# liulab-dfci/TRUST4

Measured on AMD Instinct MI355X. Metric: stage-1 assembly read pairs/sec (150 bp PE), whole stage 1, higher is better.
Workload: dtype int32/u64

## Files before the change

### trust4_amd/csrc/t4_api.hip

```cpp
#include <hip/hip_runtime.h>
#include <math.h>
#include <stdarg.h>
#include <stdio.h>
#include <string.h>
#include <zlib.h>

#include <algorithm>
#include <atomic>
#include <chrono>
#include <map>
#include <memory>
#include <mutex>
#include <string>
#include <thread>
#include <unordered_map>
#include <vector>

#ifdef __HIPCC__
#include <dlfcn.h>
#include <rccl/rccl.h>
#include <type_traits>
#include <unistd.h>
#endif
#include "../../include/trust4_hip.h"
// ... 293 lines not shown
    while (n < groups) n *= 2;
    if (c->grpPoolHost) (void)hipHostFree(c->grpPoolHost);
    c->grpPoolHost = nullptr; w.grpPool = nullptr; w.grpCap = 0;
    HIPCHK(c, hipHostMalloc(&c->grpPoolHost, sizeof(T4Grp) * 2 * (size_t)n, hipHostMallocMapped));
    HIPCHK(c, hipHostGetDevicePointer((void **)&w.grpPool, c->grpPoolHost, 0));
    w.grpCap = n;
  }
  return T4_OK;
}
T4Wide wideHalf(const t4_ctx *c, int half) {
  T4Wide w = c->wide;
  if (!half) return w;
  const size_t R = (size_t)w.maxReads, P = (size_t)w.maxPart;
  w.seed += R * T4_WIDE_SEEDS; w.bounds += R * (T4_WIDE_MAXP + 1); w.uniqPref += R * (w.pcap + 1); w.sortTmp += R * 2 * w.pcap; w.requeue += R; w.headBits += R * ((w.pcap + 31) / 32);
  w.pCnt += P; w.pRead += P; w.pKeys += P * w.pcap; w.gSize += P * w.pcap; w.gInfo += P * w.pcap; w.gCount += P * 4; w.gOff += P * 2;
  w.pRec += P * w.maxOvPart * 10; w.pRecCnt += P; w.mKeys += P * w.maxOvPart; w.mOrd += P * w.maxOvPart;
  w.grpPool += w.grpCap;
  return w;
}

}

extern "C" {

int t4_init(int device_ordinal, t4_ctx **out) {
  if (!out) return T4_ERR_ARG;
  *out = nullptr;
  int ndev = 0;
  if (hipGetDeviceCount(&ndev) != hipSuccess || ndev <= 0 || device_ordinal < 0 || device_ordinal >= ndev) return T4_ERR_HIP;
  if (hipSetDevice(device_ordinal) != hipSuccess) return T4_ERR_HIP;
  t4_ctx *c = new t4_ctx();
  c->device = device_ordinal;
  hipDeviceProp_t prop;
  if (hipGetDeviceProperties(&prop, device_ordinal) != hipSuccess) { delete c; return T4_ERR_HIP; }
  c->cus = prop.multiProcessorCount;
  if (hipStreamCreate(&c->stream) != hipSuccess) { delete c; return T4_ERR_HIP; }
  for (int i = 0; i < 4; ++i) if (hipEventCreate(&c->ev[i]) != hipSuccess) { delete c; return T4_ERR_HIP; }
  memset(&c->stats, 0, sizeof c->stats);
  if (hipMalloc(&c->listCounts, sizeof(int) * 16) != hipSuccess || hipMalloc(&c->hitCounter, sizeof(unsigned long long)) != hipSuccess) { delete c; return T4_ERR_HIP; }
  if (hipHostMalloc(&c->aqFlagHost, 64, hipHostMallocMapped) != hipSuccess || hipHostGetDevicePointer((void **)&c->aqFlagDev, c->aqFlagHost, 0) != hipSuccess ||
      hipMalloc(&c->aqDoneCtr, sizeof(unsigned)) != hipSuccess || hipMemset(c->aqDoneCtr, 0, sizeof(unsigned)) != hipSuccess) { delete c; return T4_ERR_HIP; }
  *c->aqFlagHost = 0;
  *out = c;
  return T4_OK;
}

void t4_destroy(t4_ctx *c) {
  if (!c) return;
  (void)hipSetDevice(c->device);
#ifdef T4_PHASE_TIMING
  if (getenv("T4_PHASE_DUMP")) {
    unsigned long long ph[T4_NPHASE];
    if (hipMemcpyFromSymbol(ph, HIP_SYMBOL(t4k::g_phaseCycles), sizeof(ph)) == hipSuccess) {
      static const char *names[32] = {"other", "seed:lookup", "expand", "sort", "stats", "runs", "bigsort", "chain", "ovsort", "score", "prefilter", "final", "annotate", "score:quick", "score:banded", "score:finish", "extend:ungapped", "after-extend", "extend:list", "extend:dp4", "extend:dp1", "extend:combine", "seed:replay", "seed:scan", "extend:launch", "-", "-", "-", "-", "-", "-", "-"};
      unsigned long long tot = 0;
      for (int i = 0; i < T4_NPHASE; ++i) tot += ph[i];
      for (int i = 0; i < T4_NPHASE; ++i) if (ph[i]) fprintf(stderr, "phase %-16s %-7s %6.2f%%  %.3e cycles\n", names[i & 31], i < 32 ? "lds" : "global", 100.0 * (double)ph[i] / (double)tot, (double)ph[i]);
    }
    static unsigned long long cls[4 * T4_NPHASE];
    if (hipMemcpyFromSymbol(cls, HIP_SYMBOL(t4k::g_phaseByOverlaps), sizeof(cls)) == hipSuccess) {
      static const char *names[32] = {"other", "seed:lookup", "expand", "sort", "stats", "runs", "bigsort", "chain", "ovsort", "score", "prefilter", "final", "annotate", "score:quick", "score:banded", "score:finish", "extend:ungapped", "after-extend", "extend:list", "extend:dp4", "extend:dp1", "extend:combine", "seed:replay", "seed:scan", "extend:launch", "-", "-", "-", "-", "-", "-", "-"};
      static const char *cname[4] = {"<5 overlaps", "5-19 overlaps", "20-64 overlaps", ">64 overlaps"};
      for (int k = 0; k < 4; ++k) {
        unsigned long long tot = 0;
        for (int i = 0; i < T4_NPHASE; ++i) tot += cls[k * T4_NPHASE + i];
        if (!tot) continue;
        fprintf(stderr, "AddRead queries with %s: %.3e cycles in the query kernel\n", cname[k], (double)tot);
        for (int i = 0; i < T4_NPHASE; ++i) if (cls[k * T4_NPHASE + i] * 200 >= tot) fprintf(stderr, "   %-16s %-7s %6.2f%%\n", names[i & 31], i < 32 ? "lds" : "global", 100.0 * (double)cls[k * T4_NPHASE + i] / (double)tot);
      }
    }
    unsigned long long dc[8];
    if (hipMemcpyFromSymbol(dc, HIP_SYMBOL(t4k::g_dbgCount), sizeof(dc)) == hipSuccess)
      fprintf(stderr, "debug counters: gap jobs %llu, banded %llu, wave-DP steps %llu, scratch fallbacks %llu; overhang DPs %llu, of which %llu leave the diagonal\n", dc[0], dc[1], dc[2], dc[3], dc[6], dc[7]);
  }
#endif
  void *ptrs[] = {c->dpRows, c->dpDir, c->gKeys, c->gPairs, c->gCand, c->gOv, c->gFin, c->gOrd, c->hitsKeys, c->lists,
                  c->listCounts, c->status, c->counts, c->hitCounter, c->result, c->aqIn, c->aqOut};
  if (c->aqInHost) (void)hipHostFree(c->aqInHost);
  if (c->aqOutHost) (void)hipHostFree(c->aqOutHost);
  if (c->aqFlagHost) (void)hipHostFree(c->aqFlagHost);
  if (c->aqDoneCtr) (void)hipFree(c->aqDoneCtr);
  if (c->aqPool) (void)hipHostFree(c->aqPool);
  if (c->candPool) (void)hipHostFree(c->candPool);
  if (c->aqRecDev) (void)hipFree(c->aqRecDev);
  if (c->aqRecRead) (void)hipFree(c->aqRecRead);
  if (c->aqExtAux) (void)hipFree(c->aqExtAux);
  if (c->wideInit) {
    void *wp[] = {c->wide.seed, c->wide.bounds, c->wide.pCnt, c->wide.pRead, c->wide.pKeys, c->wide.gSize, c->wide.gInfo, c->wide.gCount, c->wide.gOff, c->wide.pRec,
                  c->wide.pRecCnt, c->wide.uniqPref, c->wide.mKeys, c->wide.mOrd, c->wide.sortTmp, c->wide.requeue};
    for (void *p : wp) if (p) (void)hipFree(p);
    if (c->grpPoolHost) (void)hipHostFree(c->grpPoolHost);
    if (c->headBitsHost) (void)hipHostFree(c->headBitsHost);
  }
  for (void *p : ptrs) if (p) (void)hipFree(p);
  for (int i = 0; i < 4; ++i) if (c->ev[i]) (void)hipEventDestroy(c->ev[i]);
  if (c->stream) (void)hipStreamDestroy(c->stream);
  if (c->stream2) (void)hipStreamDestroy(c->stream2);
  if (c->evIn) (void)hipEventDestroy(c->evIn);
  if (c->evG) (void)hipEventDestroy(c->evG);
  delete c;
}

int t4_sync(t4_ctx *c) {
  if (!c) return T4_ERR_ARG;
  HIPCHK(c, hipStreamSynchronize(c->stream));
  return T4_OK;
}
const char *t4_last_error(t4_ctx *c) { return c ? c->err.c_str() : "null ctx"; }
int t4_device_cus(t4_ctx *c) { return c ? c->cus : 0; }
int t4_ctx_device(t4_ctx *c) { return c ? c->device : 0; }
#ifdef T4_PHASE_TIMING
int t4_debug_phase_cycles(unsigned long long *out16) {
  unsigned long long zero[T4_NPHASE] = {0};
  if (hipMemcpyFromSymbol(out16, HIP_SYMBOL(t4k::g_phaseCycles), sizeof(zero)) != hipSuccess) return T4_ERR_HIP;
// ... 2696 lines not shown
```

### trust4_amd/csrc/t4_kernels.h

```cpp
#pragma once
#include <hip/hip_runtime.h>

#include "t4_device.h"

namespace t4k {

#ifdef T4_INLINE_ALL
#define T4_NI
#else
#define T4_NI __attribute__((noinline))
#endif
#ifndef T4_OPT_JOBSORT
#define T4_OPT_JOBSORT 1
#endif
#ifndef T4_OPT_ROWWALK
#define T4_OPT_ROWWALK 1
#endif
#ifndef T4_NI_R3
#define T4_NI_R3 0
#endif
#ifdef __HIPCC__
#define T4_LDS_AS __attribute__((address_space(3)))
#else
#define T4_LDS_AS
// ... 2737 lines not shown
    if (f == i) {
      slotOf[i] = k;
      if (gt == 3 && cSlot < 0) cSlot = k;
      kept[k++] = oi;
    } else if (f < i && gt == 2) {
      const int used = slotOf[f];
      const OvRec &base = wm.fin[kept[used]];
      if (o.matchCnt == base.matchCnt && ovSimDen(o) == ovSimDen(base) && cSlot >= 0) {
        const OvRec &c = wm.fin[kept[cSlot]];
        if (o.re <= c.rs + 3) {
          int d1 = o.re - c.rs, d2 = base.re - c.rs;
          if (d1 < 0) d1 = -d1;
          if (d2 < 0) d2 = -d2;
          if (base.re > c.rs + 3 || d1 < d2) kept[used] = oi;
        }
      }
    }
  }
  if (k > 0) {
    char BT = 0, chain = 0;
    for (int i = 0; i < k; ++i) {
      const OvRec &o = wm.fin[kept[i]];
      char n0 = OV_NAME0(o.flags), n2 = OV_NAME2(o.flags);
      if (BT && n0 != BT) continue;
      BT = n0;
      if (chain && !(n2 == chain || (n2 == 'D' && chain == 'A') || (n2 == 'A' && chain == 'D'))) continue;
      chain = n2;
      int gt = OV_GENETYPE(o.flags) == 255 ? -1 : OV_GENETYPE(o.flags);
      if (gt >= 0 && g[gt] == -1) g[gt] = kept[i];
    }
    if (g[3] != -1) {
      const OvRec &c = wm.fin[g[3]];
      if (c.re - c.rs + 1 <= readLen / 2 && c.re - c.rs + 1 <= 50) {
        for (int i = 0; i < 3; ++i) {
          if (g[i] < 0) continue;
          const OvRec &x = wm.fin[g[i]];
          if ((x.re - 17 > c.rs || c.re < x.re) && c.ss >= 100) { g[3] = -1; break; }
        }
      }
    }
  }
  for (int t = 0; t < 4; ++t) {
    if (g[t] >= 0) storeOverlap(out + t, wm.fin[g[t]]);
    else {
      T4OverlapOut z;
      z.seqIdx = -1; z.readStart = z.readEnd = z.seqStart = z.seqEnd = -1; z.strand = 1; z.matchCnt = 0; z.indelCnt = 0; z.similarity = 0;
      out[t] = z;
    }
  }
}

struct ExtSide { short size, good, match, mis, indel, pending; };
struct ExtOut { int ret, rs, re, ss, se, matchCnt, simFail, den; };

#define T4_EXT_BYTES(L) (((L) + 1) * 11 + 3 * (L) + 8)
#define T4_EXT_WST(buf, L) ((buf) + ((L) + 1) * 11 + 2 * (L) + 8)
#define PS_INDEL (1u << 27)
__device__ __forceinline__ unsigned pathStepDiag(unsigned s, bool eq) {
  if (s & PS_INDEL) return s;
  unsigned good = s & 511u, tmp = (s >> 9) & 511u, k = ((s >> 18) & 511u) + 1u;
  if (eq) { ++tmp; if (4u * tmp > 3u * k) good = k; }
  return good | tmp << 9 | k << 18;
}
__device__ __forceinline__ unsigned pathBorder(int n) {
  const unsigned one = 1u | 1u << 9 | 1u << 18;
  return n == 1 ? one : (one | PS_INDEL);
}
__device__ unsigned dpWaveTracePW(const T4PW *w, int L, const char *p, unsigned char *dirbuf) {
  const int d = laneId(), W = 11, leftBand = 5;
  unsigned char *wst = T4_EXT_WST(dirbuf, L);
  for (int t = d; t < L; t += 64) wst[t] = w[t];
  waveLdsSync();
  const int negInf = (L + 1) * (L + 1) * (-4);
  int M = negInf;
  unsigned S = PS_INDEL, fin = PS_INDEL;
  { int j0 = d - leftBand; if (d < W && j0 >= 0 && j0 <= L) M = j0 == 0 ? 0 : -4 - 4 * j0; }
  const int lastStep = 2 * L + W - 1;
  for (int s = 2; s <= lastStep; ++s) {
    int lM = waveUp1(M), uM = waveDown1(M);
    const unsigned lS = waveUp1(S), uS = waveDown1(S);
    const int i2 = s - d, i = i2 >> 1, j = i - leftBand + d;
    if (d < W && (i2 & 1) == 0 && i >= 1 && i <= L && j >= 1 && j <= L) {
      if (j == 1) lM = -4 - 4 * i; else if (d == 0) lM = negInf;
      if (i == 1) uM = -4 - 4 * j; else if (d + 1 >= W) uM = negInf;
      int dM;
      if (i == 1) dM = (j - 1 == 0) ? 0 : -4 - 4 * (j - 1);
      else if (j == 1) dM = -4 - 4 * (i - 1);
      else dM = M;
      const bool eq = baseEqualW(wst[j - 1], p[i - 1]);
      const int dsc = dM + (eq ? 2 : -2);
      int m = dsc;
      if (lM - 4 > m) m = lM - 4;
      if (uM - 4 > m) m = uM - 4;
      dirbuf[i * W + d] = (unsigned char)((lM - 4 == m ? 1 : 0) | (uM - 4 == m ? 2 : 0) | (dsc == m ? 4 : 0) | (eq ? 8 : 0));
      if (dsc == m) S = pathStepDiag((i == 1 && j == 1) ? 0u : ((i == 1 || j == 1) ? pathBorder(i + j - 2) : S), eq);
      else if (uM - 4 == m) S = (i == 1 ? pathBorder(j) : uS) | PS_INDEL;
      else S = (j == 1 ? pathBorder(i) : lS) | PS_INDEL;
      if (i == L && j == L) fin = S;
      M = m;
    }
  }
  return (unsigned)__shfl((int)fin, leftBand);
}
__device__ unsigned dpRowTracePW(const T4PW *w, int L, const char *p, unsigned char *dirbuf, int Lmax) {
  const int d = laneId() & 15, W = 11, leftBand = 5;
  unsigned char *wst = T4_EXT_WST(dirbuf, L);
// ... 56 lines not shown
      if (i == 1) uM = -4 - 4 * j; else if (last) uM = (neg_);                                                                         \
      const int dM = i == 1 ? (j == 1 ? 0 : -4 * j) : (j == 1 ? -4 * i : Mself);                                                       \
      const bool eq = baseEqualW((w_)[j - 1], (p_)[i - 1]);                                                                            \
      const int dsc = dM + (eq ? 2 : -2);                                                                                              \
      int m = dsc;                                                                                                                     \
      if (lM - 4 > m) m = lM - 4;                                                                                                      \
      if (uM - 4 > m) m = uM - 4;                                                                                                      \
      if (dsc == m) { Sself = pathStepDiag((i == 1 && j == 1) ? 0u : ((i == 1 || j == 1) ? pathBorder(i + j - 2) : Sself), eq); Rself = (i == 1 ? 0 : Rself) + 1; } \
      else if (uM - 4 == m) { Sself = (i == 1 ? pathBorder(j) : uS) | PS_INDEL; Rself = 0; }                                           \
      else { Sself = (j == 1 ? pathBorder(i) : lS) | PS_INDEL; Rself = 0; }                                                            \
      Mself = m;                                                                                                                       \
    }                                                                                                                                  \
  }
  for (int u = 0; u < nPair; ++u) {
    T4_PAIR_STEP(ME, MO, SE, SO, RE, LE, wE, pE, negE, iE)
    T4_PAIR_STEP(MO, ME, SO, SE, RO, LO, wO, pO, negO, iO)
    ++iE; ++iO;
  }
#undef T4_PAIR_STEP
  const int src = (laneId() & ~15) + leftBand;
  const unsigned sA = (unsigned)__shfl((int)SO, src), sB = (unsigned)__shfl((int)SE, src);
  const unsigned rA = (unsigned)__shfl(RO, src), rB = (unsigned)__shfl(RE, src);
  outA = (unsigned long long)sA | ((unsigned long long)rA << 32);
  outB = (unsigned long long)sB | ((unsigned long long)rB << 32);
}
__device__ int tracebackPW(const unsigned char *dirbuf, int L, signed char *align) {
  const int W = 11, leftBand = 5;
  int tagi = L, tagj = L, tag = 0;
  while (tagi > 0 || tagj > 0) {
    int a = 0;
    if (tagi > 0 && tagj > 0) {
      unsigned char bits = dirbuf[tagi * W + (tagj - tagi + leftBand)];
      if (bits & 1) a = 3;
      if (bits & 2) a = 2;
      if (bits & 4) a = (bits & 8) ? 0 : 1;
    } else if (tagi == 0) {
      int mL = (tagj - 1 == 0) ? 0 : (-4 - 4 * (tagj - 1));
      if (mL - 4 == -4 - 4 * tagj) a = 3;
    } else {
      int mU = (tagi - 1 == 0) ? 0 : (-4 - 4 * (tagi - 1));
      if (mU - 4 == -4 - 4 * tagi) a = 2;
    }
    align[tag++] = (signed char)a;
    if (a == 3) --tagj; else if (a == 2) --tagi; else { --tagi; --tagj; }
  }
  for (int i = 0, j = tag - 1; i < j; ++i, --j) { signed char x = align[i]; align[i] = align[j]; align[j] = x; }
  return tag;
}

__device__ void extendOverlaps(const T4IndexView &ix, WaveMem &wm, WaveState *ws, int n, int len, bool useFirstStrand,
                               double factor, ExtSide *sides, unsigned char *dirbuf, int dirBytes, ExtOut *res, bool lean = false) {
  const int lane = tid(), NT = nthr();
  const int plus0 = n > 0 ? (wm.fin[wm.ord[0]].flags & OV_PLUS) : 1;
  {
    const int wave = lane >> 6, nwv = NT >> 6, wl = lane & 63;
    for (int q = wave; q < 2 * n; q += nwv) {
      const OvRec &o = wm.fin[wm.ord[q >> 1]];
      const int side = q & 1;
      const T4SeqInfo si = ix.seqs[o.seqIdx];
      const char *r = (useFirstStrand ? plus0 : (o.flags & OV_PLUS)) ? wm.seg : wm.rc;
      int size, t0, p0;
      if (side == 0) { size = o.rs < o.ss ? o.rs : o.ss; t0 = o.ss - size; p0 = o.rs - size; }
      else { int a = len - 1 - o.re, b = si.len - 1 - o.se; size = a < b ? a : b; t0 = o.se + 1; p0 = o.re + 1; }
      const T4PW *w = ix.pw + si.pwOff + t0;
      int mm = 0, good = 0, tmpBase = 0;
      for (int base = 0; base < size; base += 64) {
        const int k = base + wl;
        const int pos = side == 0 ? size - 1 - k : k;
        const bool in = k < size;
        const bool eq = in && baseEqualW(w[pos], r[p0 + pos]);
        const unsigned long long bal = __ballot(eq);
        const int tmp = tmpBase + __popcll(bal & ((wl == 63) ? ~0ull : ((2ull << wl) - 1ull)));
        const unsigned long long gb = __ballot(eq && tmp > 0.75 * (k + 1));
        if (gb) good = base + 64 - __clzll((long long)gb);
        mm += __popcll(__ballot(in && !eq));
        tmpBase += __popcll(bal);
      }
      if (wl == 0) {
        ExtSide e;
        e.size = (short)size; e.match = (short)(size - mm); e.mis = (short)mm; e.indel = 0; e.pending = 0;
        if (size > 1 && !((size - mm) * 2 - mm * 2 >= size * 2 - 8)) e.pending = 1;
        e.good = (short)good;
        sides[q] = e;
      }
    }
  }
  __syncthreads();
  PHASE_MARK(ws, 18);
  if (lean) {
    int nPend = 0, maxL = 0;
    for (int q0 = 0; q0 < 2 * n; q0 += NT) {
      const int q = q0 + lane;
      const bool pend = q < 2 * n && sides[q].pending;
      int tot;
      const int inc = blockInclScan(pend ? 1 : 0, ws->red, tot);
      if (pend) wm.cand[nPend + inc - 1] = (unsigned)q;
      nPend += tot;
      int mx;
      blockInclMaxScan(pend ? (int)sides[q].size : 0, ws->red, mx);
      if (mx > maxL) maxL = mx;
    }
    __syncthreads();
    PHASE_MARK(ws, 19);
    const int nw = NT >> 6, slice = (maxL + 15) & ~15;
    int perChunk = nw * 8;
    if (slice > 0 && perChunk * slice > dirBytes) perChunk = (dirBytes / slice) & ~7;
    if (nPend > 0 && perChunk < 8) { if (lane == 0) ws->unsupported = 1; nPend = 0; }
    const int wave = lane >> 6, wl = lane & 63, row = wl >> 4, l16 = wl & 15;
    for (int c0 = 0; c0 < nPend; c0 += perChunk) {
      int Lq[2] = {0, 0}, qq[2] = {-1, -1};
      const unsigned char *wst[2] = {dirbuf, dirbuf};
      const char *pr[2] = {wm.seg, wm.seg};
      for (int z = 0; z < 2; ++z) {
        const int slot = wave * 8 + row * 2 + z, t = c0 + slot;
        if (slot < perChunk && t < nPend) {
          const int q = (int)wm.cand[t];
          const OvRec &o = wm.fin[wm.ord[q >> 1]];
          const int side = q & 1, L = sides[q].size;
          const T4SeqInfo si = ix.seqs[o.seqIdx];
          const char *r = (useFirstStrand ? plus0 : (o.flags & OV_PLUS)) ? wm.seg : wm.rc;
          const T4PW *w = ix.pw + si.pwOff + (side == 0 ? o.ss - L : o.se + 1);
          unsigned char *dst = dirbuf + (size_t)slot * slice;
          for (int x = l16; x < L; x += 16) dst[x] = w[x];
          Lq[z] = L; qq[z] = q; wst[z] = dst; pr[z] = r + (side == 0 ? o.rs - L : o.re + 1);
        }
      }
      waveLdsSync();
      int Lmax = Lq[0] > Lq[1] ? Lq[0] : Lq[1];
      { int x = __shfl_xor(Lmax, 16); if (x > Lmax) Lmax = x; x = __shfl_xor(Lmax, 32); if (x > Lmax) Lmax = x; }
      unsigned long long out[2];
      dpRowPairLean(wst[0], Lq[0], pr[0], wst[1], Lq[1], pr[1], Lmax, out[0], out[1]);
      for (int z = 0; z < 2; ++z) {
        const bool have = qq[z] >= 0;
        const unsigned pst = (unsigned)out[z];
        const int q = have ? qq[z] : 0, side = q & 1, L = Lq[z];
        const bool gapped = have && (pst & PS_INDEL) != 0;
        DBG_ADD(6, (have && l16 == 0) ? 1 : 0); DBG_ADD(7, (gapped && l16 == 0) ? 1 : 0);
        const int run = (gapped && side == 0) ? (int)(out[z] >> 32) : 0;
        int runMax = run;
        { int x = __shfl_xor(runMax, 16); if (x > runMax) runMax = x; x = __shfl_xor(runMax, 32); if (x > runMax) runMax = x; }
        int good = 0, tmpBase = 0;
        for (int base = 0; base < runMax; base += 16) {
          const int k = base + l16;
          const bool eq = k < run && baseEqualW(wst[z][L - 1 - k], pr[z][L - 1 - k]);
          const unsigned bal = (unsigned)((__ballot(eq) >> (wl & 48)) & 0xFFFFull);
          const int tmp = tmpBase + __popc(bal & ((2u << l16) - 1u));
          const unsigned gb = (unsigned)((__ballot(eq && 4 * tmp > 3 * (k + 1)) >> (wl & 48)) & 0xFFFFull);
          if (gb) good = base + 32 - __clz(gb);
          tmpBase += __popc(bal);
        }
        if (gapped && side == 1) good = (int)(pst & 511u);
        if (have && l16 == 0) {
          ExtSide e = sides[q];
          if (gapped) { e.match = 0; e.mis = 0; e.indel = 1; e.good = (short)good; }
          e.pending = 0;
          sides[q] = e;
        }
      }
      __syncthreads();
    }
    PHASE_MARK(ws, 21);
  } else {
  const int nwE = NT >> 6, perChunk = nwE * 4;
  const int qslice = (dirBytes / perChunk) & ~15;
  int nFit = 0, nPendSides = 0;
  for (int part = 0; part < 2; ++part) {
    for (int q0 = 0; q0 < 2 * n; q0 += NT) {
      const int q = q0 + lane;
      bool pend = q < 2 * n && sides[q].pending;
      if (pend) { const int size = sides[q].size; const bool fitsQ = T4_EXT_BYTES(size) <= qslice; pend = (part == 0) == fitsQ; }
      int tot;
      const int inc = blockInclScan(pend ? 1 : 0, ws->red, tot);
      if (pend) wm.cand[nPendSides + inc - 1] = (unsigned)q;
      nPendSides += tot;
    }
    if (part == 0) nFit = nPendSides;
  }
  __syncthreads();
  auto finishSide = [&](int q, const signed char *align, int alen) {
    const int side = q & 1;
    int m = 0, mm = 0, ind = 0, good = 0, tmp = 0;
    for (int k = 0; k < alen; ++k) { if (align[k] == 0) ++m; else if (align[k] == 1) ++mm; else ++ind; }
    if (side == 0) {
      for (int i = alen - 1, k = 1; i >= 0; --i, ++k) {
        if (align[i] == 0) { ++tmp; if (tmp > 0.75 * k) good = k; }
        else if (align[i] != 1) break;
      }
    } else {
      for (int i = 0; i < alen; ++i) {
        if (align[i] == 0) { ++tmp; if (tmp > 0.75 * (i + 1)) good = i + 1; }
        else if (align[i] != 1) break;
      }
    }
    ExtSide e = sides[q];
    e.match = (short)m; e.mis = (short)mm; e.indel = (short)ind; e.good = (short)good; e.pending = 0;
    sides[q] = e;
  };
  auto leanSide = [&](int q, const unsigned char *buf, int L, signed char *align) {
    const int side = q & 1;
    int good = 0, tmp = 0;
    if (side == 0) {
      const int W = 11, leftBand = 5;
      int tagi = L, tagj = L, k = 0;
      while (tagi > 0 && tagj > 0) {
        const unsigned char bits = buf[tagi * W + (tagj - tagi + leftBand)];
        if (!(bits & 4)) break;
        ++k;
        if (bits & 8) { ++tmp; if (tmp > 0.75 * k) good = k; }
        --tagi; --tagj;
      }
    } else {
      const int alen = tracebackPW(buf, L, align);
      for (int i = 0; i < alen; ++i) {
        if (align[i] == 0) { ++tmp; if (tmp > 0.75 * (i + 1)) good = i + 1; }
        else if (align[i] != 1) break;
// ... 521 lines not shown
    if (VARIANT == 2) {
      if (SHARED_ARGS) { __syncthreads(); if (threadIdx.x == 0) s_ix = qa.views[qa.viewOf[r]]; __syncthreads(); }
      else ix = qa.views[qa.viewOf[r]];
    }
#ifdef __HIPCC__
    const unsigned long long tick0 = (VARIANT == 1 && qa.readTicks) ? wall_clock64() : 0ull;
#endif
    bool done = processRead<(VARIANT == 0 ? 0 : VARIANT == 3 ? 3 : 1)>(ix, bv, wk, qa, wm, &s_ws, r, sc);
    if (CAP == 8192 && VARIANT == 1 && !done && wk.gKeys) {
      WaveMem wgLocal;
      WaveMem &wg = SHARED_ARGS ? s_wg : wgLocal;
      __syncthreads();
      if (!SHARED_ARGS || threadIdx.x == 0) {
        wg = wm;
        const size_t b = blockIdx.x;
        wg.keys = wk.gKeys + b * (size_t)wk.gCap;
        wg.pairs = wk.gPairs + b * (size_t)wk.gCap * 2;
        wg.cand = wg.pairs + wk.gCap;
        wg.ov = (OvRec *)(wk.gOv + b * (size_t)wk.gMaxOv * 10);
        wg.fin = (OvRec *)(wk.gFin + b * (size_t)wk.gMaxOv * 10);
        wg.ord = wk.gOrd + b * (size_t)wk.gMaxOv;
        wg.cap = wk.gCap; wg.maxOv = wk.gMaxOv; wg.maxFin = wk.gMaxOv; wg.candCap = wk.gCap; wg.ldsArrays = 0; wg.hitLimit = wk.gCap;
        wg.ldsSort = s_keys; wg.ldsSortCap = C;
        wg.dirBuf = (unsigned char *)s_keys; wg.dirBytes = C * 8;
        if (wk.capLimit > 0 && wk.capLimit < C) { int bsz = 64; while (bsz * 2 <= wk.capLimit) bsz *= 2; wg.ldsSortCap = bsz; }
      }
      __syncthreads();
      done = processRead<1>(ix, bv, wk, qa, wg, &s_ws, r, sc);
      if (tid() == 0 && done && wk.nextCount) atomicAdd(wk.nextCount + 2, 1);
    }
    if (tid() == 0) {
#ifdef __HIPCC__
      if (VARIANT == 1 && qa.readTicks) qa.readTicks[r] = (int)(wall_clock64() - tick0);
#endif
#ifdef T4_PHASE_TIMING
      if (VARIANT == 1 && qa.mode == 4) {
        const int nOv = qa.counts[r], cls = nOv < 5 ? 0 : nOv < 20 ? 1 : nOv <= 64 ? 2 : 3;
        for (int p_ = 0; p_ < T4_NPHASE; ++p_) if (s_ws.phaseLocal[p_]) { atomicAdd(&g_phaseByOverlaps[cls * T4_NPHASE + p_], (unsigned long long)s_ws.phaseLocal[p_]); s_ws.phaseLocal[p_] = 0; }
      }
#endif
      if (!done) {
        if (wk.nextList) { int slot = atomicAdd(wk.nextCount, 1); wk.nextList[slot] = (int)r; }
        else wk.status[r] = 2;
      }
      s_nextW = wk.workNext ? (int)gridDim.x + atomicAdd(wk.workNext, 1) : w + (int)gridDim.x;
    }
    __syncthreads();
    w = s_nextW;
    __syncthreads();
  }
}

#ifndef T4_EXT_NREC
#define T4_EXT_NREC 4
#endif
__global__ __launch_bounds__(64) void extendKernel(T4IndexView ix, T4BatchView bv, T4QueryArgs qa, int recBegin) {
  __shared__ OvRec s_fin[T4_EXT_NREC];
  __shared__ unsigned short s_ord[T4_EXT_NREC];
  __shared__ ExtSide s_sides[2 * T4_EXT_NREC];
  __shared__ ExtOut s_res[T4_EXT_NREC];
  __shared__ unsigned s_cand[2 * T4_EXT_NREC + 2];
  __shared__ unsigned long long s_dir[1024];
  __shared__ char s_seg[T4_MAXL + 8];
  __shared__ char s_rc[T4_MAXL + 8];
  __shared__ WaveState s_ws;
  WaveMem wm;
  wm.keys = s_dir; wm.pairs = (unsigned *)s_sides; wm.ov = (OvRec *)s_res; wm.fin = s_fin; wm.ord = s_ord; wm.cand = s_cand;
  wm.seg = s_seg; wm.rc = s_rc;
  wm.cap = 1024; wm.maxOv = T4_EXT_NREC; wm.maxFin = T4_EXT_NREC; wm.candCap = 2 * T4_EXT_NREC + 2; wm.ldsArrays = 1;
  wm.ldsSort = nullptr; wm.ldsSortCap = 0; wm.hitLimit = 0; wm.dirBuf = (unsigned char *)s_dir; wm.dirBytes = (int)sizeof s_dir;
  const int lane = tid();
  const int nRec = (int)*qa.poolCursor < qa.poolCap ? (int)*qa.poolCursor : qa.poolCap;
  for (int g = recBegin + (int)blockIdx.x * T4_EXT_NREC; g < nRec; g += (int)gridDim.x * T4_EXT_NREC) {
    int i0 = g;
    const int gEnd = g + T4_EXT_NREC < nRec ? g + T4_EXT_NREC : nRec;
    while (i0 < gEnd) {
      const int r = qa.recRead[i0];
      int i1 = i0 + 1;
      while (i1 < gEnd && qa.recRead[i1] == r) ++i1;
      if (r < 0) { i0 = i1; continue; }
      const int n = i1 - i0, len = bv.len[r];
      if (lane == 0) { s_ws.overflow = 0; s_ws.unsupported = 0; }
#ifdef T4_PHASE_TIMING
      if (lane == 0) { s_ws.phaseT0 = clock64(); s_ws.phaseBase = 0; s_ws.curPhase = 24; }
#endif
      loadSegment(bv, r, 0, len, wm);
      if (lane < n) {
        const T4OverlapOut t = qa.outDev[i0 + lane];
        OvRec o;
        o.seqIdx = t.seqIdx; o.rs = t.readStart; o.re = t.readEnd; o.ss = t.seqStart; o.se = t.seqEnd;
        o.matchCnt = t.matchCnt; o.indelCnt = t.indelCnt; o.chainPos = 0; o.chainLen = 0;
        o.flags = t.strand == 1 ? OV_PLUS : 0;
        s_fin[lane] = o; s_ord[lane] = (unsigned short)lane;
      }
      __syncthreads();
      extendOverlaps(ix, wm, &s_ws, n, len, false, qa.factorPerRead[r], s_sides, (unsigned char *)s_dir, (int)sizeof s_dir, s_res, qa.leanExt != 0);
      if (lane < n) {
        const T4OverlapOut in = qa.outDev[i0 + lane];
        const ExtOut e = s_res[lane];
        T4OverlapOut t;
        t.seqIdx = in.seqIdx; t.readStart = e.rs; t.readEnd = e.re; t.seqStart = e.ss; t.seqEnd = e.se;
        t.strand = in.strand; t.matchCnt = e.matchCnt;
        if (e.simFail) { t.indelCnt = in.indelCnt; t.similarity = in.similarity; }
        else { t.indelCnt = 0; t.similarity = (double)t.matchCnt / (double)e.den; }
        qa.outExt[i0 + lane] = t;
        qa.ret[i0 + lane] = e.ret;
        if (qa.cs && qa.cs->extAux) qa.cs->extAux[i0 + lane] = e.simFail ? 0 : e.den;
      }
      if (lane == 0 && s_ws.unsupported) qa.poolCursor[1] = 1u;
      __syncthreads();
      i0 = i1;
    }
  }
}

struct PickBest { int idx, seqIdx, rs, re, ss, se, matchCnt, flags; };
__device__ __forceinline__ OvRec pickRec(const PickBest &b) {
  OvRec o;
  o.seqIdx = b.seqIdx; o.rs = b.rs; o.re = b.re; o.ss = b.ss; o.se = b.se; o.matchCnt = b.matchCnt; o.indelCnt = 0; o.chainPos = 0; o.chainLen = 0; o.flags = b.flags;
  return o;
}
__device__ __forceinline__ PickBest pickLoad(const T4OverlapOut *ov, int i) {
  const T4OverlapOut t = ov[i];
  PickBest b;
  b.idx = i; b.seqIdx = t.seqIdx; b.rs = t.readStart; b.re = t.readEnd; b.ss = t.seqStart; b.se = t.seqEnd; b.matchCnt = t.matchCnt;
  b.flags = (t.strand == 1 ? OV_PLUS : 0) | (t.similarity == 0 ? OV_SIMZERO : 0);
  return b;
}
__device__ __forceinline__ bool pickBefore(const PickBest &a, const PickBest &b) {
  const int cm = ovCmp(pickRec(a), pickRec(b), true);
  return cm < 0 || (cm == 0 && a.idx < b.idx);
}
__device__ __forceinline__ PickBest pickShflXor(const PickBest &b, int d) {
  PickBest o;
  o.idx = __shfl_xor(b.idx, d); o.seqIdx = __shfl_xor(b.seqIdx, d); o.rs = __shfl_xor(b.rs, d); o.re = __shfl_xor(b.re, d);
  o.ss = __shfl_xor(b.ss, d); o.se = __shfl_xor(b.se, d); o.matchCnt = __shfl_xor(b.matchCnt, d); o.flags = __shfl_xor(b.flags, d);
  return o;
}
__device__ __forceinline__ PickBest pickReduce(PickBest b, bool wantLast, PickBest *red) {
  for (int d = 32; d > 0; d >>= 1) {
    const PickBest o = pickShflXor(b, d);
    if (o.idx >= 0 && (b.idx < 0 || pickBefore(o, b) != wantLast)) b = o;
  }
  const int wave = threadIdx.x >> 6, nw = (blockDim.x + 63) >> 6;
  if (laneId() == 0) red[wave] = b;
  __syncthreads();
  b = red[0];
  for (int w = 1; w < nw; ++w) {
    const PickBest o = red[w];
    if (o.idx >= 0 && (b.idx < 0 || pickBefore(o, b) != wantLast)) b = o;
  }
  __syncthreads();
  return b;
}
#define T4_PICK_THREADS 256
__global__ __launch_bounds__(T4_PICK_THREADS) void assignPickKernel(int nReads, const int *counts, const int *outBase, const int *lens,
                                                                    const T4OverlapOut *ov, const T4OverlapOut *ext, const int *ret, const int *extAux,
                                                                    int poolCap, int *outRet, T4OverlapOut *out) {
  __shared__ PickBest s_red[T4_PICK_THREADS / 64];
  const int lane = tid(), NT = nthr();
  for (int r = blockIdx.x; r < nReads; r += gridDim.x) {
    const int len = lens[r];
    int n = counts[r], base = n > 0 ? outBase[r] : 0;
    if (n < 0 || base < 0 || base > poolCap) n = 0;
    if (n > poolCap - base) n = poolCap - base;
// ... 637 lines not shown
```

### trust4_amd/csrc/t4_wide.h

```cpp
#pragma once

#define T4_WIDE_SEEDS (2 * T4_MAXL + 2)
#define T4_WIDE_OVBITS 9
#define T4_WIDE_PART_SAMPLES 256

__device__ T4_NI void wideDeferRead(const T4IndexView &ix, WaveMem &wm, WaveState *ws, const T4Wide &wd, int len, int strandArg, long long r,
                                    unsigned long long &hitTotal, int pass, int barcode) {
  const int lane = tid(), NT = nthr();
  unsigned *posStart = (unsigned *)wm.ov, *posPref = wm.pairs;
  const int nk = len - ix.k + 1;
  __syncthreads();
  const int H = seedPositionsNovel(ix, wm, len, strandArg, barcode, pass == 1, posStart, posPref, ws->red, wm.keys, (WaveState *)0);
  hitTotal += (unsigned long long)H;
  int huge = 0;
  if (barcode == -1) for (int q = lane; q < 2 * nk; q += NT) if (posPref[q + 1] - posPref[q] > 10000u) huge = 1;
  huge = blockSum(huge, ws->red) != 0;
  if (lane == 0) {
    int slot = atomicAdd(&wd.ctl[0], 1), pBase = 0, P = 0;
    if (slot >= wd.maxReads) { atomicOr(&wd.ctl[2], 1); slot = -1; }
    else {
      const long long per = 16LL * wd.pcap;
      long long want = ((long long)H * wd.safetyNum + per - 1) / per;
      const int nseq = ix.nseq > 0 ? ix.nseq : 1;
      if (want < 1) want = 1;
// ... 389 lines not shown
      run += tot;
    }
    if (lane == 0) { up[0] = 0; st[WS_M] = lim; }
    __syncthreads();
    unsigned *hb = wd.headBits + (size_t)w * ((wd.pcap + 31) / 32);
    for (int j = lane; j < (lim + 31) / 32; j += NT) {
      unsigned v = 0;
      for (int b = 0; b < 32 && j * 32 + b < lim; ++b) v |= (unsigned)(up[j * 32 + b + 1] - up[j * 32 + b]) << b;
      hb[j] = v;
    }
  }
}

template <int PCAP, int MAXOV>
__global__ __launch_bounds__(512) void wideChainKernel(T4IndexView ixArg, T4BatchView bvArg, T4Work wkArg, T4QueryArgs qaArg, T4Wide wd) {
  __shared__ unsigned long long s_keys[PCAP];
  __shared__ unsigned s_pairs[PCAP + PCAP / 3 + 2];
  __shared__ OvRec s_ov[MAXOV];
  __shared__ unsigned short s_ord[MAXOV];
  __shared__ char s_seg[T4_MAXL + 8];
  __shared__ char s_rc[T4_MAXL + 8];
  __shared__ WaveState s_ws;
  __shared__ T4IndexView s_ix;
  __shared__ T4BatchView s_bv;
  __shared__ T4Work s_wk;
  __shared__ T4QueryArgs s_qa;
  __shared__ WaveMem s_wm;
  if (wd.ctl[2]) return;
  if (threadIdx.x == 0) {
    s_ix = ixArg; s_bv = bvArg; s_wk = wkArg; s_qa = qaArg;
    WaveMem &m = s_wm;
    m.keys = s_keys; m.pairs = s_pairs; m.cand = s_pairs + PCAP; m.ov = s_ov; m.fin = s_ov; m.ord = s_ord;
    m.cap = PCAP; m.maxOv = MAXOV; m.maxFin = MAXOV; m.candCap = PCAP / 3 + 2; m.ldsArrays = 1; m.hitLimit = PCAP;
    m.ldsSort = nullptr; m.ldsSortCap = 0; m.dirBuf = (unsigned char *)s_keys; m.dirBytes = PCAP * 8;
    m.seg = s_seg; m.rc = s_rc;
  }
  __syncthreads();
  const T4IndexView &ix = s_ix;
  const T4BatchView &bv = s_bv;
  const T4Work &wk = s_wk;
  WaveMem &wm = s_wm;
  WaveState *ws = &s_ws;
  DPScratch sc;
  sc.rows = wk.dpRows + ((size_t)blockIdx.x * (blockDim.x >> 6) + (threadIdx.x >> 6)) * (6 * T4_ROWW * 64);
  sc.dir = wk.dpDir + ((size_t)blockIdx.x * blockDim.x + threadIdx.x) * T4_DIR_BYTES;
  const int nPart = wideParts(wd), lane = threadIdx.x, NT = blockDim.x, K = ix.k;
  for (int pg = wd.firstPart + blockIdx.x; pg < nPart; pg += gridDim.x) {
    const int w = wd.pRead[pg];
    const T4WidePlan pl = wd.plan[w];
    const int n = (int)wd.pCnt[pg];
    __syncthreads();
    if (lane == 0) { ws->overflow = 0; ws->unsupported = 0; ws->finCount = 0; ws->ovCount = 0; ws->candCount = 0; ws->jobCount = 0; ws->statsStable = 1; ws->wideWant = 0; }
    if (n == 0) continue;
    const long long r = pl.read;
    const int len = bv.len[r];
    loadSegment(bv, r, 0, len, wm);
    const unsigned long long *gk = wd.pKeys + (size_t)pg * wd.pcap;
    for (int i = lane; i < n; i += NT) s_keys[i] = gk[i];
    const int *st = wd.stat + (size_t)w * T4_WIDE_STAT;
    if (lane == 0) { ws->novelMin[0] = st[WS_NOVELMIN]; ws->novelMin[1] = st[WS_NOVELMIN + 1]; }
    const int ror0 = st[WS_ROR], ror1 = st[WS_ROR + 1], M = st[WS_M];
    __syncthreads();
    unsigned *gs = wm.pairs;
    int nG = 0;
    for (int i0 = 0; i0 < n; i0 += NT) {
      const int i = i0 + lane;
      const bool stt = i < n && (i == 0 || KEY_G(s_keys[i]) != KEY_G(s_keys[i - 1]));
      int tot;
      const int inc = blockInclScan(stt ? 1 : 0, ws->red, tot);
      if (stt) gs[nG + inc - 1] = (unsigned)i;
      nG += tot;
    }
    __syncthreads();
    {
      const int *gc = wd.gCount + (size_t)pg * 4;
      const int nMinus = gc[0];
      const int off0 = wd.gOff[(size_t)pg * 2], off1 = wd.gOff[(size_t)pg * 2 + 1];
      T4Grp *out = wd.grpPool + pl.grpBase;
      for (int g = lane; g < nG; g += NT) {
        const int s0 = (int)gs[g], e0 = g + 1 < nG ? (int)gs[g + 1] : n;
        int lo = 0x7FFFFFFF, hi = -0x7FFFFFFF;
        for (int i = s0; i < e0;) {
          const int c = KEY_C(s_keys[i]);
          int j = i + 1;
          while (j < e0 && KEY_C(s_keys[j]) == c) ++j;
          if (j - i >= 3) {
            const int at = -(c - T4_C_BIAS);
            if (at < lo) lo = at;
            if (at + len - 1 > hi) hi = at + len - 1;
          }
          i = j;
        }
        const unsigned long long k0 = s_keys[s0];
        T4Grp rec;
        rec.key = (unsigned)KEY_IDX(k0) * 2u + (unsigned)KEY_PLUS(k0); rec.cnt = (unsigned)(e0 - s0); rec.lo = lo; rec.hi = hi;
        if (pl.huge) rec.cnt |= (unsigned)wd.gInfo[(size_t)pg * wd.pcap + g] << 24;
        out[g < nMinus ? off0 + g : off1 + (g - nMinus)] = rec;
      }
    }
    __syncthreads();
    unsigned *starts = wm.pairs;
    int nRuns = 0;
    for (int i0 = 0; i0 < n; i0 += NT) {
      const int i = i0 + lane;
      bool runStart = false;
      if (i < n) {
// ... 258 lines not shown
```

Before: 18900.

## Stage reference windows into LDS before ungapped extension and batch extend records

The ungapped extension in extendOverlaps now first writes per-side staging records, then cooperatively copies each side's reference window from global memory into LDS using 16-lane rows with four loads in flight, and runs the match scan from LDS with 16-lane groups instead of one wave per side. The lean DP path reuses these staged windows rather than reloading them. extendKernel now loads all record metadata for a group in one pass, and the records per block drop from 4 to 2. This aims to hide global-memory latency and cut redundant loads, at the cost of more barriers, LDS capacity limits that can mark reads unsupported, and less work per block.

```diff
diff --git a/trust4_amd/csrc/t4_api.hip b/trust4_amd/csrc/t4_api.hip
--- a/trust4_amd/csrc/t4_api.hip
+++ b/trust4_amd/csrc/t4_api.hip
@@ -369,14 +369,14 @@
   if (getenv("T4_PHASE_DUMP")) {
     unsigned long long ph[T4_NPHASE];
     if (hipMemcpyFromSymbol(ph, HIP_SYMBOL(t4k::g_phaseCycles), sizeof(ph)) == hipSuccess) {
-      static const char *names[32] = {"other", "seed:lookup", "expand", "sort", "stats", "runs", "bigsort", "chain", "ovsort", "score", "prefilter", "final", "annotate", "score:quick", "score:banded", "score:finish", "extend:ungapped", "after-extend", "extend:list", "extend:dp4", "extend:dp1", "extend:combine", "seed:replay", "seed:scan", "extend:launch", "-", "-", "-", "-", "-", "-", "-"};
+      static const char *names[32] = {"other", "seed:lookup", "expand", "sort", "stats", "runs", "bigsort", "chain", "ovsort", "score", "prefilter", "final", "annotate", "score:quick", "score:banded", "score:finish", "extend:ungapped", "after-extend", "extend:list", "extend:dp4", "extend:dp1", "extend:combine", "seed:replay", "seed:scan", "extK:ungapped", "-", "extK:list", "extK:stage", "extK:dp", "extK:combine", "-", "extK:prologue"};
       unsigned long long tot = 0;
       for (int i = 0; i < T4_NPHASE; ++i) tot += ph[i];
       for (int i = 0; i < T4_NPHASE; ++i) if (ph[i]) fprintf(stderr, "phase %-16s %-7s %6.2f%%  %.3e cycles\n", names[i & 31], i < 32 ? "lds" : "global", 100.0 * (double)ph[i] / (double)tot, (double)ph[i]);
     }
     static unsigned long long cls[4 * T4_NPHASE];
     if (hipMemcpyFromSymbol(cls, HIP_SYMBOL(t4k::g_phaseByOverlaps), sizeof(cls)) == hipSuccess) {
-      static const char *names[32] = {"other", "seed:lookup", "expand", "sort", "stats", "runs", "bigsort", "chain", "ovsort", "score", "prefilter", "final", "annotate", "score:quick", "score:banded", "score:finish", "extend:ungapped", "after-extend", "extend:list", "extend:dp4", "extend:dp1", "extend:combine", "seed:replay", "seed:scan", "extend:launch", "-", "-", "-", "-", "-", "-", "-"};
+      static const char *names[32] = {"other", "seed:lookup", "expand", "sort", "stats", "runs", "bigsort", "chain", "ovsort", "score", "prefilter", "final", "annotate", "score:quick", "score:banded", "score:finish", "extend:ungapped", "after-extend", "extend:list", "extend:dp4", "extend:dp1", "extend:combine", "seed:replay", "seed:scan", "extK:ungapped", "-", "extK:list", "extK:stage", "extK:dp", "extK:combine", "-", "extK:prologue"};
       static const char *cname[4] = {"<5 overlaps", "5-19 overlaps", "20-64 overlaps", ">64 overlaps"};
       for (int k = 0; k < 4; ++k) {
         unsigned long long tot = 0;
diff --git a/trust4_amd/csrc/t4_kernels.h b/trust4_amd/csrc/t4_kernels.h
--- a/trust4_amd/csrc/t4_kernels.h
+++ b/trust4_amd/csrc/t4_kernels.h
@@ -2813,6 +2813,8 @@
 
 struct ExtSide { short size, good, match, mis, indel, pending; };
 struct ExtOut { int ret, rs, re, ss, se, matchCnt, simFail, den; };
+struct ExtStg { long long pw; short p0, size, plus, pad; };
+static_assert(2 * sizeof(ExtStg) == sizeof(ExtOut), "ExtStg: the staging records of an overlap's two sides live in its ExtOut");
 
 #define T4_EXT_BYTES(L) (((L) + 1) * 11 + 3 * (L) + 8)
 #define T4_EXT_WST(buf, L) ((buf) + ((L) + 1) * 11 + 2 * (L) + 8)
@@ -2975,31 +2977,68 @@
                                double factor, ExtSide *sides, unsigned char *dirbuf, int dirBytes, ExtOut *res, bool lean = false) {
   const int lane = tid(), NT = nthr();
   const int plus0 = n > 0 ? (wm.fin[wm.ord[0]].flags & OV_PLUS) : 1;
-  {
-    const int wave = lane >> 6, nwv = NT >> 6, wl = lane & 63;
-    for (int q = wave; q < 2 * n; q += nwv) {
+  typedef T4_LDS_AS unsigned char *LdsW;
+  typedef const T4_LDS_AS char *LdsR;
+  ExtStg *const stg = (ExtStg *)res;
+  const int wave = lane >> 6, nw = NT >> 6, wl = lane & 63, row = wl >> 4, l16 = wl & 15, grow = lane >> 4, nrow = NT >> 4;
+  const int stride = len > 16 ? (len + 15) & ~15 : 16;
+  const int perStage = dirBytes / stride;
+  if (perStage < 1) { if (lane == 0) ws->unsupported = 1; n = 0; }
+  for (int qa = 0; qa < 2 * n; qa += perStage) {
+    const int qb = qa + perStage < 2 * n ? qa + perStage : 2 * n;
+    for (int q = qa + lane; q < qb; q += NT) {
       const OvRec &o = wm.fin[wm.ord[q >> 1]];
-      const int side = q & 1;
       const T4SeqInfo si = ix.seqs[o.seqIdx];
-      const char *r = (useFirstStrand ? plus0 : (o.flags & OV_PLUS)) ? wm.seg : wm.rc;
       int size, t0, p0;
-      if (side == 0) { size = o.rs < o.ss ? o.rs : o.ss; t0 = o.ss - size; p0 = o.rs - size; }
+      if ((q & 1) == 0) { size = o.rs < o.ss ? o.rs : o.ss; t0 = o.ss - size; p0 = o.rs - size; }
       else { int a = len - 1 - o.re, b = si.len - 1 - o.se; size = a < b ? a : b; t0 = o.se + 1; p0 = o.re + 1; }
-      const T4PW *w = ix.pw + si.pwOff + t0;
-      int mm = 0, good = 0, tmpBase = 0;
-      for (int base = 0; base < size; base += 64) {
-        const int k = base + wl;
+      ExtStg g;
+      g.pw = (long long)si.pwOff + t0; g.p0 = (short)p0; g.size = (short)size;
+      g.plus = (short)((useFirstStrand ? plus0 : (o.flags & OV_PLUS)) ? 1 : 0); g.pad = 0;
+      stg[q] = g;
+    }
+    __syncthreads();
+    for (int q = qa + grow; q < qb; q += nrow) {
+      const ExtStg g = stg[q];
+      const T4PW *w = ix.pw + g.pw;
+      const LdsW dst = (LdsW)dirbuf + (q - qa) * stride;
+      const int size = g.size < stride ? g.size : stride;
+      for (int x0 = l16; x0 < size; x0 += 64) {
+        T4PW v[4];
+#pragma unroll
+        for (int u = 0; u < 4; ++u) v[u] = x0 + 16 * u < size ? w[x0 + 16 * u] : (T4PW)0;
+#pragma unroll
+        for (int u = 0; u < 4; ++u) if (x0 + 16 * u < size) dst[x0 + 16 * u] = v[u];
+      }
+    }
+    __syncthreads();
+    for (int q0 = qa; q0 < qb; q0 += nrow) {
+      const int q = q0 + grow, side = q & 1;
+      const bool have = q < qb;
+      int size = 0;
+      LdsW w = (LdsW)dirbuf;
+      LdsR r = (LdsR)wm.seg;
+      if (have) {
+        const ExtStg g = stg[q];
+        size = g.size < stride ? g.size : stride;
+        w = (LdsW)dirbuf + (q - qa) * stride;
+        r = (LdsR)(g.plus ? wm.seg : wm.rc) + g.p0;
+      }
+      int smax = size;
+      { int x = __shfl_xor(smax, 16); if (x > smax) smax = x; x = __shfl_xor(smax, 32); if (x > smax) smax = x; }
+      int good = 0, tmpBase = 0;
+      for (int base = 0; base < smax; base += 16) {
+        const int k = base + l16;
         const int pos = side == 0 ? size - 1 - k : k;
-        const bool in = k < size;
-        const bool eq = in && baseEqualW(w[pos], r[p0 + pos]);
-        const unsigned long long bal = __ballot(eq);
-        const int tmp = tmpBase + __popcll(bal & ((wl == 63) ? ~0ull : ((2ull << wl) - 1ull)));
-        const unsigned long long gb = __ballot(eq && tmp > 0.75 * (k + 1));
-        if (gb) good = base + 64 - __clzll((long long)gb);
-        mm += __popcll(__ballot(in && !eq));
-        tmpBase += __popcll(bal);
-      }
-      if (wl == 0) {
+        const bool eq = k < size && baseEqualW(w[pos], r[pos]);
+        const unsigned bal = (unsigned)((__ballot(eq) >> (wl & 48)) & 0xFFFFull);
+        const int tmp = tmpBase + __popc(bal & ((2u << l16) - 1u));
+        const unsigned gb = (unsigned)((__ballot(eq && 4 * tmp > 3 * (k + 1)) >> (wl & 48)) & 0xFFFFull);
+        if (gb) good = base + 32 - __clz(gb);
+        tmpBase += __popc(bal);
+      }
+      if (have && l16 == 0) {
+        const int mm = (size > 0 ? size : 0) - tmpBase;
         ExtSide e;
         e.size = (short)size; e.match = (short)(size - mm); e.mis = (short)mm; e.indel = 0; e.pending = 0;
         if (size > 1 && !((size - mm) * 2 - mm * 2 >= size * 2 - 8)) e.pending = 1;
@@ -3007,48 +3046,34 @@
         sides[q] = e;
       }
     }
-  }
-  __syncthreads();
-  PHASE_MARK(ws, 18);
-  if (lean) {
-    int nPend = 0, maxL = 0;
-    for (int q0 = 0; q0 < 2 * n; q0 += NT) {
+    __syncthreads();
+    if (!lean) continue;
+    PHASE_MARK(ws, 18);
+    int nPend = 0;
+    for (int q0 = qa; q0 < qb; q0 += NT) {
       const int q = q0 + lane;
-      const bool pend = q < 2 * n && sides[q].pending;
+      const bool pend = q < qb && sides[q].pending;
       int tot;
       const int inc = blockInclScan(pend ? 1 : 0, ws->red, tot);
       if (pend) wm.cand[nPend + inc - 1] = (unsigned)q;
       nPend += tot;
-      int mx;
-      blockInclMaxScan(pend ? (int)sides[q].size : 0, ws->red, mx);
-      if (mx > maxL) maxL = mx;
     }
     __syncthreads();
     PHASE_MARK(ws, 19);
-    const int nw = NT >> 6, slice = (maxL + 15) & ~15;
-    int perChunk = nw * 8;
-    if (slice > 0 && perChunk * slice > dirBytes) perChunk = (dirBytes / slice) & ~7;
-    if (nPend > 0 && perChunk < 8) { if (lane == 0) ws->unsupported = 1; nPend = 0; }
-    const int wave = lane >> 6, wl = lane & 63, row = wl >> 4, l16 = wl & 15;
-    for (int c0 = 0; c0 < nPend; c0 += perChunk) {
+    for (int c0 = 0; c0 < nPend; c0 += nw * 8) {
+      const bool onePerRow = nPend - c0 <= nw * 4;
       int Lq[2] = {0, 0}, qq[2] = {-1, -1};
       const unsigned char *wst[2] = {dirbuf, dirbuf};
       const char *pr[2] = {wm.seg, wm.seg};
       for (int z = 0; z < 2; ++z) {
-        const int slot = wave * 8 + row * 2 + z, t = c0 + slot;
-        if (slot < perChunk && t < nPend) {
+        const int t = c0 + (onePerRow ? wave * 4 + row : wave * 8 + row * 2 + z);
+        if (t < nPend && !(onePerRow && z)) {
           const int q = (int)wm.cand[t];
-          const OvRec &o = wm.fin[wm.ord[q >> 1]];
-          const int side = q & 1, L = sides[q].size;
-          const T4SeqInfo si = ix.seqs[o.seqIdx];
-          const char *r = (useFirstStrand ? plus0 : (o.flags & OV_PLUS)) ? wm.seg : wm.rc;
-          const T4PW *w = ix.pw + si.pwOff + (side == 0 ? o.ss - L : o.se + 1);
-          unsigned char *dst = dirbuf + (size_t)slot * slice;
-          for (int x = l16; x < L; x += 16) dst[x] = w[x];
-          Lq[z] = L; qq[z] = q; wst[z] = dst; pr[z] = r + (side == 0 ? o.rs - L : o.re + 1);
-        }
-      }
-      waveLdsSync();
+          const ExtStg g = stg[q];
+          Lq[z] = sides[q].size; qq[z] = q; wst[z] = dirbuf + (size_t)(q - qa) * stride; pr[z] = (g.plus ? wm.seg : wm.rc) + g.p0;
+        }
+      }
+      PHASE_MARK(ws, 20);
       int Lmax = Lq[0] > Lq[1] ? Lq[0] : Lq[1];
       { int x = __shfl_xor(Lmax, 16); if (x > Lmax) Lmax = x; x = __shfl_xor(Lmax, 32); if (x > Lmax) Lmax = x; }
       unsigned long long out[2];
@@ -3082,8 +3107,9 @@
       }
       __syncthreads();
     }
-    PHASE_MARK(ws, 21);
-  } else {
+  }
+  PHASE_MARK(ws, lean ? 21 : 18);
+  if (!lean) {
   const int nwE = NT >> 6, perChunk = nwE * 4;
   const int qslice = (dirBytes / perChunk) & ~15;
   int nFit = 0, nPendSides = 0;
@@ -3711,7 +3737,7 @@
 }
 
 #ifndef T4_EXT_NREC
-#define T4_EXT_NREC 4
+#define T4_EXT_NREC 2
 #endif
 __global__ __launch_bounds__(64) void extendKernel(T4IndexView ix, T4BatchView bv, T4QueryArgs qa, int recBegin) {
   __shared__ OvRec s_fin[T4_EXT_NREC];
@@ -3719,6 +3745,8 @@
   __shared__ ExtSide s_sides[2 * T4_EXT_NREC];
   __shared__ ExtOut s_res[T4_EXT_NREC];
   __shared__ unsigned s_cand[2 * T4_EXT_NREC + 2];
+  __shared__ int s_rr[T4_EXT_NREC], s_len[T4_EXT_NREC];
+  __shared__ double s_fac[T4_EXT_NREC], s_sim[T4_EXT_NREC];
   __shared__ unsigned long long s_dir[1024];
   __shared__ char s_seg[T4_MAXL + 8];
   __shared__ char s_rc[T4_MAXL + 8];
@@ -3731,45 +3759,53 @@
   const int lane = tid();
   const int nRec = (int)*qa.poolCursor < qa.poolCap ? (int)*qa.poolCursor : qa.poolCap;
   for (int g = recBegin + (int)blockIdx.x * T4_EXT_NREC; g < nRec; g += (int)gridDim.x * T4_EXT_NREC) {
-    int i0 = g;
-    const int gEnd = g + T4_EXT_NREC < nRec ? g + T4_EXT_NREC : nRec;
-    while (i0 < gEnd) {
-      const int r = qa.recRead[i0];
+    const int cnt = g + T4_EXT_NREC < nRec ? T4_EXT_NREC : nRec - g;
+    const int rr = lane < cnt ? qa.recRead[g + lane] : -1;
+    if (rr >= 0) {
+      const T4OverlapOut in = qa.outDev[g + lane];
+      s_len[lane] = bv.len[rr];
+      s_fac[lane] = qa.factorPerRead[rr];
+      OvRec o;
+      o.seqIdx = in.seqIdx; o.rs = in.readStart; o.re = in.readEnd; o.ss = in.seqStart; o.se = in.seqEnd;
+      o.matchCnt = in.matchCnt; o.indelCnt = in.indelCnt; o.chainPos = 0; o.chainLen = 0;
+      o.flags = in.strand == 1 ? OV_PLUS : 0;
+      s_fin[lane] = o; s_sim[lane] = in.similarity;
+    }
+    if (lane < T4_EXT_NREC) { s_ord[lane] = (unsigned short)lane; s_rr[lane] = rr; }
+    __syncthreads();
+    for (int i0 = 0; i0 < cnt;) {
+      const int r = s_rr[i0];
       int i1 = i0 + 1;
-      while (i1 < gEnd && qa.recRead[i1] == r) ++i1;
+      while (i1 < cnt && s_rr[i1] == r) ++i1;
       if (r < 0) { i0 = i1; continue; }
-      const int n = i1 - i0, len = bv.len[r];
+      const int n = i1 - i0, len = s_len[i0];
+      const double factor = s_fac[i0];
       if (lane == 0) { s_ws.overflow = 0; s_ws.unsupported = 0; }
 #ifdef T4_PHASE_TIMING
-      if (lane == 0) { s_ws.phaseT0 = clock64(); s_ws.phaseBase = 0; s_ws.curPhase = 24; }
+      if (lane == 0) { s_ws.phaseT0 = clock64(); s_ws.phaseBase = 8; s_ws.curPhase = 31; }
 #endif
+      wm.fin = s_fin + i0;
       loadSegment(bv, r, 0, len, wm);
-      if (lane < n) {
-        const T4OverlapOut t = qa.outDev[i0 + lane];
-        OvRec o;
-        o.seqIdx = t.seqIdx; o.rs = t.readStart; o.re = t.readEnd; o.ss = t.seqStart; o.se = t.seqEnd;
-        o.matchCnt = t.matchCnt; o.indelCnt = t.indelCnt; o.chainPos = 0; o.chainLen = 0;
-        o.flags = t.strand == 1 ? OV_PLUS : 0;
-        s_fin[lane] = o; s_ord[lane] = (unsigned short)lane;
-      }
-      __syncthreads();
-      extendOverlaps(ix, wm, &s_ws, n, len, false, qa.factorPerRead[r], s_sides, (unsigned char *)s_dir, (int)sizeof s_dir, s_res, qa.leanExt != 0);
-      if (lane < n) {
-        const T4OverlapOut in = qa.outDev[i0 + lane];
-        const ExtOut e = s_res[lane];
+      PHASE_MARK(&s_ws, 16);
+      extendOverlaps(ix, wm, &s_ws, n, len, false, factor, s_sides, (unsigned char *)s_dir, (int)sizeof s_dir, s_res, qa.leanExt != 0);
+      if (lane >= i0 && lane < i1) {
+        const ExtOut e = s_res[lane - i0];
+        const OvRec in = s_fin[lane];
         T4OverlapOut t;
         t.seqIdx = in.seqIdx; t.readStart = e.rs; t.readEnd = e.re; t.seqStart = e.ss; t.seqEnd = e.se;
-        t.strand = in.strand; t.matchCnt = e.matchCnt;
-        if (e.simFail) { t.indelCnt = in.indelCnt; t.similarity = in.similarity; }
+        t.strand = (in.flags & OV_PLUS) ? 1 : -1; t.matchCnt = e.matchCnt;
+        if (e.simFail) { t.indelCnt = in.indelCnt; t.similarity = s_sim[lane]; }
         else { t.indelCnt = 0; t.similarity = (double)t.matchCnt / (double)e.den; }
-        qa.outExt[i0 + lane] = t;
-        qa.ret[i0 + lane] = e.ret;
-        if (qa.cs && qa.cs->extAux) qa.cs->extAux[i0 + lane] = e.simFail ? 0 : e.den;
+        qa.outExt[g + lane] = t;
+        qa.ret[g + lane] = e.ret;
+        if (qa.cs && qa.cs->extAux) qa.cs->extAux[g + lane] = e.simFail ? 0 : e.den;
       }
       if (lane == 0 && s_ws.unsupported) qa.poolCursor[1] = 1u;
       __syncthreads();
+      PHASE_MARK(&s_ws, 23);
       i0 = i1;
     }
+    __syncthreads();
   }
 }
 
diff --git a/trust4_amd/csrc/t4_wide.h b/trust4_amd/csrc/t4_wide.h
--- a/trust4_amd/csrc/t4_wide.h
+++ b/trust4_amd/csrc/t4_wide.h
@@ -465,6 +465,9 @@
     __syncthreads();
     if (lane == 0) { ws->overflow = 0; ws->unsupported = 0; ws->finCount = 0; ws->ovCount = 0; ws->candCount = 0; ws->jobCount = 0; ws->statsStable = 1; ws->wideWant = 0; }
     if (n == 0) continue;
+#ifdef T4_PHASE_TIMING
+    if (lane == 0) { ws->phaseT0 = clock64(); ws->phaseBase = 32; ws->curPhase = 32; }
+#endif
     const long long r = pl.read;
     const int len = bv.len[r];
     loadSegment(bv, r, 0, len, wm);
```

Measured after the change: 17010. 10.0% lower.
